# zju3dv/pvnet

Measured on NVIDIA H100. Metric: images/sec (480x640, K=9) backbone+vote, higher is better.
Workload: dtype tf32 (fp32 storage, fp32 accumulate; vote fp32/fp64)

## Files before the change

pvnet_b200/csrc/conv_tc.cu:

```cuda
#include "conv_tc.cuh"
#include "ptx.cuh"

#include <cstdlib>
#include <mutex>
#include <new>

namespace pvnet {

struct ConvGeom {
    int Ho, Wo;
    int tiles_x, tiles_y, total_m_tiles;
    int TH, TW;
    int taps, cin_chunks, cin_pad;
    int Cout, BN;
    int out_cs, out_co;
    int res_cs, res_co;
    int act;
    int round_out;
    signed char tap_map[9];
    short tap_ox[9], tap_oy[9];
    int n_items;
    int stages;
};

struct AMaps {
    CUtensorMap m[4];
};

constexpr int CONV_THREADS = 288;
constexpr int CONV_KC = 32;
constexpr int CONV_A_BYTES = 128 * CONV_KC * 4;

template <int BN, bool MC>
__global__ void __launch_bounds__(CONV_THREADS, 1)
    k_conv_tap(const __grid_constant__ AMaps amaps, const __grid_constant__ CUtensorMap tmB, const __grid_constant__ ConvGeom g,
               const float *__restrict__ bias, const float *__restrict__ res, float *__restrict__ out)
{
    constexpr int B_BYTES = BN * CONV_KC * 4;
    constexpr int STAGE_BYTES = CONV_A_BYTES + B_BYTES;
    const int STAGES = g.stages;
    extern __shared__ uint8_t smem_raw[];
    uint8_t *smem = reinterpret_cast<uint8_t *>((reinterpret_cast<uintptr_t>(smem_raw) + 1023) & ~uintptr_t(1023));
    uint64_t *full = reinterpret_cast<uint64_t *>(smem + (size_t)STAGES * STAGE_BYTES);
    uint64_t *empty = full + STAGES;

    const int warp = threadIdx.x >> 5, lane = threadIdx.x & 31;
    const int tiles_per_img = g.tiles_x * g.tiles_y;
    const int n_tiles_n = g.Cout / BN;
    const int nkb = g.taps * g.cin_chunks;
    const uint32_t crank = MC ? ptx::cluster_ctarank() : 0u;
    const int unit = MC ? (int)blockIdx.x >> 1 : (int)blockIdx.x, nunits = MC ? (int)gridDim.x >> 1 : (int)gridDim.x;
    auto item_tile = [&](int item, int &m_tile, int &n0) {
        const int mi = item / n_tiles_n;
        n0 = (item - mi * n_tiles_n) * BN;
        m_tile = MC ? min(2 * mi + (int)crank, g.total_m_tiles - 1) : mi;
    };

    if (threadIdx.x == 0) {
        for (int s = 0; s < STAGES; ++s) {
            ptx::mbar_init(&full[s], 1);
            ptx::mbar_init(&empty[s], MC ? 16 : 8);
        }
        ptx::fence_barrier_init();
    }
    __syncthreads();
    if (MC) ptx::cluster_sync();

    if (warp == 8) {
        if (lane == 0) {
            int s = 0;
            uint32_t ph = 0;
            for (int item = unit; item < g.n_items; item += nunits) {
                int m_tile, n0;
                item_tile(item, m_tile, n0);
                const int img = m_tile / tiles_per_img;
                const int trem = m_tile - img * tiles_per_img;
                const int tyi = trem / g.tiles_x, txi = trem - tyi * g.tiles_x;
                const int y0 = tyi * g.TH, x0 = txi * g.TW;
                for (int tap = 0; tap < g.taps; ++tap)
                    for (int cc = 0; cc < g.cin_chunks; ++cc) {
                        ptx::mbar_wait(&empty[s], ph ^ 1u);
                        ptx::mbar_arrive_expect_tx(&full[s], (uint32_t)STAGE_BYTES);
                        uint8_t *sa = smem + (size_t)s * STAGE_BYTES;
                        ptx::tma_load_4d(sa, &amaps.m[g.tap_map[tap]], &full[s], cc * CONV_KC, x0 + g.tap_ox[tap],
                                         y0 + g.tap_oy[tap], img);
                        if (MC)
                            ptx::tma_load_2d_mc(sa + CONV_A_BYTES + crank * (B_BYTES / 2), &tmB, &full[s],
                                                tap * g.cin_pad + cc * CONV_KC, n0 + (int)crank * (BN / 2), (uint16_t)0x3);
                        else
                            ptx::tma_load_2d(sa + CONV_A_BYTES, &tmB, &full[s], tap * g.cin_pad + cc * CONV_KC, n0);
                        if (++s == STAGES) {
                            s = 0;
                            ph ^= 1u;
                        }
                    }
            }
        }
    } else {
        const int wg = warp >> 2, wq = warp & 3;
        const int g8 = lane >> 2, t4 = lane & 3;
        const uint32_t smem_u = ptx::smem_u32(smem);
        auto release = [&](int st) {
            ptx::mbar_arrive(&empty[st]);
            if (MC) ptx::mbar_arrive_cluster(&empty[st], crank ^ 1u);
        };
        int s = 0;
        uint32_t ph = 0;
        for (int item = unit; item < g.n_items; item += nunits) {
            float acc[BN / 2];
#pragma unroll
            for (int i = 0; i < BN / 2; ++i) acc[i] = 0.f;
            int prev = -1;
            for (int kb = 0; kb < nkb; ++kb) {
                ptx::mbar_wait(&full[s], ph);
                const uint32_t sa = smem_u + (uint32_t)s * (uint32_t)STAGE_BYTES;
                const uint64_t adesc = ptx::make_kmajor_desc(sa + (uint32_t)(wg * 64 * 128), 128);
                const uint64_t bdesc = ptx::make_kmajor_desc(sa + (uint32_t)CONV_A_BYTES, 128);
                ptx::wgmma_fence();
#pragma unroll
                for (int k = 0; k < CONV_KC / 8; ++k)
                    ptx::Wgmma<BN>::ss(acc, adesc + (uint64_t)(2 * k), bdesc + (uint64_t)(2 * k), (kb | k) != 0 ? 1u : 0u);
                ptx::wgmma_commit();
                ptx::wgmma_wait<1>();
                ptx::fence_regs(acc);
                if (prev >= 0 && lane == 0) release(prev);
                prev = s;
                if (++s == STAGES) {
                    s = 0;
                    ph ^= 1u;
                }
            }
            ptx::wgmma_wait<0>();
            ptx::fence_regs(acc);
            if (lane == 0) release(prev);

            int m_tile, n0;
            item_tile(item, m_tile, n0);
            const int img = m_tile / tiles_per_img;
            const int trem = m_tile - img * tiles_per_img;
            const int tyi = trem / g.tiles_x, txi = trem - tyi * g.tiles_x;
            bool ok[2];
            float *optr[2];
            const float *rptr[2];
#pragma unroll
            for (int h = 0; h < 2; ++h) {
                const int m = wg * 64 + wq * 16 + g8 + 8 * h;
                const int y = tyi * g.TH + m / g.TW, x = txi * g.TW + m % g.TW;
                ok[h] = y < g.Ho && x < g.Wo;
                const size_t pix = ok[h] ? ((size_t)img * g.Ho + y) * g.Wo + x : 0;
                optr[h] = out + pix * g.out_cs + g.out_co + n0;
                rptr[h] = res ? res + pix * g.res_cs + g.res_co + n0 : nullptr;
            }
            constexpr int JC = BN == 256 ? 2 : (BN / 8 < 8 ? BN / 8 : 8);
#pragma unroll
            for (int j0 = 0; j0 < BN / 8; j0 += JC) {
                float2 bv[JC], rv[2][JC];
#pragma unroll
                for (int jj = 0; jj < JC; ++jj)
                    bv[jj] = __ldg(reinterpret_cast<const float2 *>(bias + n0 + 8 * (j0 + jj) + 2 * t4));
                if (res) {
#pragma unroll
                    for (int h = 0; h < 2; ++h)
#pragma unroll
                        for (int jj = 0; jj < JC; ++jj)
                            rv[h][jj] = ok[h] ? __ldg(reinterpret_cast<const float2 *>(rptr[h] + 8 * (j0 + jj) + 2 * t4))
                                              : make_float2(0.f, 0.f);
                }
#pragma unroll
                for (int h = 0; h < 2; ++h) {
                    if (!ok[h]) continue;
#pragma unroll
                    for (int jj = 0; jj < JC; ++jj) {
                        const int j = j0 + jj;
                        float2 v = make_float2(acc[4 * j + 2 * h] + bv[jj].x, acc[4 * j + 2 * h + 1] + bv[jj].y);
                        if (res) {
                            v.x += rv[h][jj].x;
                            v.y += rv[h][jj].y;
                        }
                        v.x = epi_act(v.x, g.act, g.round_out);
                        v.y = epi_act(v.y, g.act, g.round_out);
                        *reinterpret_cast<float2 *>(optr[h] + 8 * j + 2 * t4) = v;
                    }
                }
            }
        }
    }
    if (MC) ptx::cluster_sync();
}

typedef CUresult (*EncodeTiledFn)(CUtensorMap *, CUtensorMapDataType, cuuint32_t, void *, const cuuint64_t *,
                                  const cuuint64_t *, const cuuint32_t *, const cuuint32_t *, CUtensorMapInterleave,
                                  CUtensorMapSwizzle, CUtensorMapL2promotion, CUtensorMapFloatOOBfill);

static EncodeTiledFn encode_fn()
{
    static EncodeTiledFn fn = nullptr;
    static std::once_flag once;
    std::call_once(once, [] {
        void *p = nullptr;
        cudaDriverEntryPointQueryResult q;
        if (cudaGetDriverEntryPoint("cuTensorMapEncodeTiled", &p, cudaEnableDefault, &q) == cudaSuccess &&
            q == cudaDriverEntryPointSuccess)
            fn = reinterpret_cast<EncodeTiledFn>(p);
    });
    return fn;
}

int tma_encode(CUtensorMap *m, const void *base, int rank, const cuuint64_t *dims, const cuuint64_t *strides_bytes,
               const cuuint32_t *box, int swizzle_bytes)
{
    EncodeTiledFn fn = encode_fn();
    if (!fn) {
        set_error("cuTensorMapEncodeTiled entry point unavailable");
        return PVNET_E_CUDA;
    }
    cuuint32_t estr[5] = {1, 1, 1, 1, 1};
    const CUtensorMapSwizzle sw = swizzle_bytes == 128 ? CU_TENSOR_MAP_SWIZZLE_128B
                                  : swizzle_bytes == 64 ? CU_TENSOR_MAP_SWIZZLE_64B
                                                        : CU_TENSOR_MAP_SWIZZLE_32B;
    CUresult r = fn(m, CU_TENSOR_MAP_DATA_TYPE_FLOAT32, (cuuint32_t)rank, const_cast<void *>(base), dims,
                    strides_bytes, box, estr, CU_TENSOR_MAP_INTERLEAVE_NONE, sw, CU_TENSOR_MAP_L2_PROMOTION_L2_128B,
                    CU_TENSOR_MAP_FLOAT_OOB_FILL_NONE);
    if (r == CUDA_ERROR_INVALID_CONTEXT || r == CUDA_ERROR_NOT_INITIALIZED) {
        cudaFree(nullptr);
        r = fn(m, CU_TENSOR_MAP_DATA_TYPE_FLOAT32, (cuuint32_t)rank, const_cast<void *>(base), dims, strides_bytes, box, estr,
               CU_TENSOR_MAP_INTERLEAVE_NONE, sw, CU_TENSOR_MAP_L2_PROMOTION_L2_128B, CU_TENSOR_MAP_FLOAT_OOB_FILL_NONE);
    }
    if (r != CUDA_SUCCESS) {
        set_error("cuTensorMapEncodeTiled failed with CUresult %d (rank %d, dims %llu %llu, box %u %u, swizzle %d)",
                  (int)r, rank, (unsigned long long)dims[0], (unsigned long long)dims[1], box[0], box[1],
                  swizzle_bytes);
        return PVNET_E_CUDA;
    }
    return PVNET_OK;
}

struct ConvPlan {
    AMaps amaps;
    CUtensorMap tmB;
    ConvGeom g;
    dim3 grid;
    size_t smem;
    int mc;
    const float *bias, *res;
    float *out;
};

int g_conv_persist = 1;
int g_conv_mc = 0;

int conv_plan(const ConvDesc &d, ConvPlan *p)
{
    PV_CHECK_ARG(d.in && d.w && d.bias && d.out, "conv: null pointer");
    PV_CHECK_ARG(!d.in2, "conv: a second input source is only supported by the column kernel");
    PV_CHECK_ARG(d.ksize == 1 || d.ksize == 3, "conv: kernel size %d unsupported", d.ksize);
    PV_CHECK_ARG(d.stride == 1 || d.stride == 2, "conv: stride %d unsupported", d.stride);
    PV_CHECK_ARG(d.stride == 1 || (d.dilation == 1 && d.H % 2 == 0 && d.W % 2 == 0),
                 "conv: stride 2 needs dilation 1 and even H,W");
    PV_CHECK_ARG(d.Cout % 32 == 0, "conv: Cout %d must be a multiple of 32", d.Cout);
    PV_CHECK_ARG(d.in_cs % 4 == 0 && d.in_co % 4 == 0 && d.out_cs % 4 == 0 && d.out_co % 4 == 0,
                 "conv: channel strides/offsets must be multiples of 4 floats");
    PV_CHECK_ARG(!d.res || (d.res_cs % 4 == 0 && d.res_co % 4 == 0), "conv: residual stride/offset alignment");
    PV_CHECK_ARG(((uintptr_t)d.in % 16 == 0) && ((uintptr_t)d.w % 16 == 0) && ((uintptr_t)d.out % 16 == 0) &&
                     ((uintptr_t)d.bias % 16 == 0),
                 "conv: pointers must be 16-byte aligned");
    PV_CHECK_ARG(d.Cin % 4 == 0, "conv: Cin %d must be a multiple of 4", d.Cin);
    const int kc = CONV_KC;
    ConvGeom &g = p->g;
    g.Ho = d.H / d.stride;
    g.Wo = d.W / d.stride;
    g.TH = 8;
    g.TW = 16;
    g.tiles_x = (g.Wo + g.TW - 1) / g.TW;
    g.tiles_y = (g.Ho + g.TH - 1) / g.TH;
    g.total_m_tiles = g.tiles_x * g.tiles_y * d.b;
    g.taps = d.ksize * d.ksize;
    g.cin_chunks = (d.Cin + kc - 1) / kc;
    g.cin_pad = g.cin_chunks * kc;
    g.Cout = d.Cout;
    {
        const long long sms = sm_count() > 0 ? sm_count() : 1;
        long long best = -1;
        for (int bn = 256; bn >= 32; bn >>= 1) {
            if (d.Cout % bn) continue;
            const long long items = (long long)g.total_m_tiles * (d.Cout / bn);
            const long long cost = (items + sms - 1) / sms * (CONV_A_BYTES + bn * kc * 4);
            if (best < 0 || cost < best) {
                best = cost;
                g.BN = bn;
            }
        }
    }
    g.out_cs = d.out_cs;
    g.out_co = d.out_co;
    g.res_cs = d.res_cs;
    g.res_co = d.res_co;
    g.act = d.act;
    g.round_out = d.round_out;
    const int pad = d.dilation * (d.ksize - 1) / 2;
    for (int t = 0; t < g.taps; ++t) {
        const int kh = t / d.ksize, kw = t - kh * d.ksize;
        if (d.stride == 1) {
            g.tap_map[t] = 0;
            g.tap_ox[t] = (short)(kw * d.dilation - pad);
            g.tap_oy[t] = (short)(kh * d.dilation - pad);
        } else {
            const int dy = kh - pad, dx = kw - pad;
            const int py = dy & 1, px = dx & 1;
            g.tap_map[t] = (signed char)(py * 2 + px);
            g.tap_oy[t] = (short)((dy - py) / 2);
            g.tap_ox[t] = (short)((dx - px) / 2);
        }
    }
    const int swz = kc * 4;
    const int nplanes = d.stride == 2 ? 4 : 1;
    for (int pl = 0; pl < nplanes; ++pl) {
        const int py = pl >> 1, px = pl & 1;
        const float *base = d.in + d.in_co + ((size_t)py * d.W + px) * d.in_cs;
        cuuint64_t dims[4] = {(cuuint64_t)d.Cin, (cuuint64_t)(d.W / d.stride), (cuuint64_t)(d.H / d.stride),
                              (cuuint64_t)d.b};
        cuuint64_t strides[3] = {(cuuint64_t)d.stride * d.in_cs * 4, (cuuint64_t)d.stride * d.W * d.in_cs * 4,
                                 (cuuint64_t)d.H * d.W * d.in_cs * 4};
        cuuint32_t box[4] = {(cuuint32_t)kc, (cuuint32_t)g.TW, (cuuint32_t)g.TH, 1};
        int rc = tma_encode(&p->amaps.m[pl], base, 4, dims, strides, box, swz);
        if (rc) return rc;
    }
    for (int pl = nplanes; pl < 4; ++pl) p->amaps.m[pl] = p->amaps.m[0];
    {
        cuuint64_t dims[2] = {(cuuint64_t)g.taps * g.cin_pad, (cuuint64_t)d.Cout};
        cuuint64_t strides[1] = {(cuuint64_t)g.taps * g.cin_pad * 4};
        p->mc = g_conv_mc;
        cuuint32_t box[2] = {(cuuint32_t)kc, (cuuint32_t)(p->mc ? g.BN / 2 : g.BN)};
        int rc = tma_encode(&p->tmB, d.w, 2, dims, strides, box, swz);
        if (rc) return rc;
    }
    const size_t stage_b = (size_t)CONV_A_BYTES + (size_t)g.BN * kc * 4;
    int st = (int)((227 * 1024 - 1024 - 256) / stage_b);
    if (st > 8) st = 8;
    g.stages = st;
    p->smem = 1024 + (size_t)st * stage_b + 256;
    const int m_units = p->mc ? (g.total_m_tiles + 1) / 2 : g.total_m_tiles;
    g.n_items = m_units * (d.Cout / g.BN);
    long long units = g_conv_persist ? (long long)sm_count() / (p->mc ? 2 : 1) : (long long)g.n_items;
    if (units > g.n_items) units = g.n_items;
    p->grid = dim3((unsigned)(units * (p->mc ? 2 : 1)));
    p->bias = d.bias;
    p->res = d.res;
    p->out = d.out;
    return PVNET_OK;
}

template <int BN, bool MC>
int conv_launch_t(const ConvPlan &p, cudaStream_t s)
{
    const cudaError_t attr_err = ensure_max_smem((const void *)k_conv_tap<BN, MC>, 227 * 1024);
    PV_CUDA(attr_err);
    cudaLaunchConfig_t cfg = {};
    cfg.gridDim = p.grid;
    cfg.blockDim = dim3(CONV_THREADS);
    cfg.dynamicSmemBytes = p.smem;
    cfg.stream = s;
    cudaLaunchAttribute attr[1];
    attr[0].id = cudaLaunchAttributeClusterDimension;
    attr[0].val.clusterDim.x = MC ? 2 : 1;
    attr[0].val.clusterDim.y = 1;
    attr[0].val.clusterDim.z = 1;
    cfg.attrs = attr;
    cfg.numAttrs = MC ? 1 : 0;
    PV_CUDA(cudaLaunchKernelEx(&cfg, k_conv_tap<BN, MC>, p.amaps, p.tmB, p.g, p.bias, p.res, p.out));
    PV_LAUNCHED("k_conv_tap");
    return PVNET_OK;
}

int conv_launch(const ConvPlan &p, cudaStream_t s)
{
    if (p.mc) {
        if (p.g.BN == 256) return conv_launch_t<256, true>(p, s);
        if (p.g.BN == 128) return conv_launch_t<128, true>(p, s);
        if (p.g.BN == 64) return conv_launch_t<64, true>(p, s);
        return conv_launch_t<32, true>(p, s);
    }
    if (p.g.BN == 256) return conv_launch_t<256, false>(p, s);
    if (p.g.BN == 128) return conv_launch_t<128, false>(p, s);
    if (p.g.BN == 64) return conv_launch_t<64, false>(p, s);
    return conv_launch_t<32, false>(p, s);
}

size_t conv_plan_size() { return sizeof(ConvPlan); }
int conv_plan_at(const ConvDesc &d, void *storage) { return conv_plan(d, new (storage) ConvPlan()); }
int conv_launch_at(const void *storage, cudaStream_t s) { return conv_launch(*static_cast<const ConvPlan *>(storage), s); }

}

extern "C" {

int pvnet_conv_set_multicast(int on)
{
    PV_CHECK_ARG(on == 0 || on == 1, "multicast mode must be 0 or 1");
    pvnet::g_conv_mc = on;
    return PVNET_OK;
}

int pvnet_conv_set_persistent(int on)
{
    pvnet::g_conv_persist = on ? 1 : 0;
    return PVNET_OK;
}

int pvnet_conv2d_nhwc(const float *in, int in_cs, int in_co, int Cin, const float *w_packed, const float *bias,
                      const float *res, int res_cs, int res_co, float *out, int out_cs, int out_co, int Cout, int b,
                      int H, int W, int ksize, int stride, int dilation, int act, int round_out,
                      pvnet_stream_t stream)
{
    pvnet::ConvDesc d{in, in_cs, in_co, Cin, w_packed, bias, res, res_cs, res_co, out, out_cs, out_co, Cout,
                      b, H, W, ksize, stride, dilation, act, round_out};
    const bool col = pvnet::g_conv_mode == 2 || (pvnet::g_conv_mode == 0 && pvnet::conv_col_eligible(d));
    if (col) {
        alignas(64) unsigned char storage[2048];
        static_assert(sizeof(storage) >= 1024, "plan storage");
        if (pvnet::conv_col_plan_size() > sizeof(storage)) {
            pvnet::set_error("column plan larger than its stack storage");
            return PVNET_E_STATE;
        }
        int rc = pvnet::conv_col_plan_at(d, nullptr, storage);
        if (rc) return rc;
        return pvnet::conv_col_launch_at(storage, (cudaStream_t)stream);
    }
    pvnet::ConvPlan plan;
    int rc = pvnet::conv_plan(d, &plan);
    if (rc) return rc;
    return pvnet::conv_launch(plan, (cudaStream_t)stream);
}

}
```

pvnet_b200/csrc/ptx.cuh:

```cuda
#pragma once
#include <cstdint>
#include <cuda.h>
#include <cuda_runtime.h>

namespace ptx {

__device__ __forceinline__ uint32_t smem_u32(const void *p)
{
    return static_cast<uint32_t>(__cvta_generic_to_shared(p));
}

__device__ __forceinline__ bool elect_one()
{
    uint32_t pred = 0;
    asm volatile(
        "{\n\t"
        ".reg .pred P1;\n\t"
        "elect.sync _|P1, 0xffffffff;\n\t"
        "selp.b32 %0, 1, 0, P1;\n\t"
        "}\n"
        : "=r"(pred));
    return pred != 0;
}

__device__ __forceinline__ void mbar_init(uint64_t *bar, uint32_t count)
{
    asm volatile("mbarrier.init.shared::cta.b64 [%0], %1;" ::"r"(smem_u32(bar)), "r"(count));
}
__device__ __forceinline__ void fence_barrier_init()
{
    asm volatile("fence.mbarrier_init.release.cluster;" ::: "memory");
}
__device__ __forceinline__ void fence_proxy_async()
{
    asm volatile("fence.proxy.async.shared::cta;" ::: "memory");
}
__device__ __forceinline__ void mbar_arrive_expect_tx(uint64_t *bar, uint32_t bytes)
{
    asm volatile("mbarrier.arrive.expect_tx.shared::cta.b64 _, [%0], %1;" ::"r"(smem_u32(bar)), "r"(bytes)
                 : "memory");
}
__device__ __forceinline__ void mbar_arrive(uint64_t *bar)
{
    asm volatile("mbarrier.arrive.shared::cta.b64 _, [%0];" ::"r"(smem_u32(bar)) : "memory");
}
__device__ __forceinline__ bool mbar_try_wait(uint64_t *bar, uint32_t parity)
{
    uint32_t ok;
    asm volatile(
        "{\n\t"
        ".reg .pred P1;\n\t"
        "mbarrier.try_wait.parity.shared::cta.b64 P1, [%1], %2;\n\t"
        "selp.b32 %0, 1, 0, P1;\n\t"
        "}\n"
        : "=r"(ok)
        : "r"(smem_u32(bar)), "r"(parity)
        : "memory");
    return ok != 0;
}
__device__ __forceinline__ void mbar_wait(uint64_t *bar, uint32_t parity)
{
    while (!mbar_try_wait(bar, parity)) {
    }
}

__device__ __forceinline__ void prefetch_tensormap(const CUtensorMap *m)
{
    asm volatile("prefetch.tensormap [%0];" ::"l"(reinterpret_cast<uint64_t>(m)) : "memory");
}
__device__ __forceinline__ void tma_load_4d(void *smem_dst, const CUtensorMap *m, uint64_t *bar, int c0, int c1,
                                            int c2, int c3)
{
    asm volatile(
        "cp.async.bulk.tensor.4d.shared::cluster.global.mbarrier::complete_tx::bytes [%0], [%1, {%3, %4, %5, %6}], [%2];"
        ::"r"(smem_u32(smem_dst)), "l"(reinterpret_cast<uint64_t>(m)), "r"(smem_u32(bar)), "r"(c0), "r"(c1), "r"(c2),
        "r"(c3)
        : "memory");
}
__device__ __forceinline__ void tma_load_2d(void *smem_dst, const CUtensorMap *m, uint64_t *bar, int c0, int c1)
{
    asm volatile(
        "cp.async.bulk.tensor.2d.shared::cluster.global.mbarrier::complete_tx::bytes [%0], [%1, {%3, %4}], [%2];"
        ::"r"(smem_u32(smem_dst)), "l"(reinterpret_cast<uint64_t>(m)), "r"(smem_u32(bar)), "r"(c0), "r"(c1)
        : "memory");
}

__device__ __forceinline__ void tma_store_4d(const CUtensorMap *m, const void *smem_src, int c0, int c1, int c2, int c3)
{
    asm volatile("cp.async.bulk.tensor.4d.global.shared::cta.bulk_group [%0, {%2, %3, %4, %5}], [%1];" ::"l"(
                     reinterpret_cast<uint64_t>(m)),
                 "r"(smem_u32(smem_src)), "r"(c0), "r"(c1), "r"(c2), "r"(c3)
                 : "memory");
}
__device__ __forceinline__ void tma_store_commit() { asm volatile("cp.async.bulk.commit_group;" ::: "memory"); }
__device__ __forceinline__ void tma_store_wait_read() { asm volatile("cp.async.bulk.wait_group.read 0;" ::: "memory"); }
__device__ __forceinline__ void tma_store_wait_read1() { asm volatile("cp.async.bulk.wait_group.read 1;" ::: "memory"); }
__device__ __forceinline__ void tma_store_wait_all() { asm volatile("cp.async.bulk.wait_group 0;" ::: "memory"); }
__device__ __forceinline__ void sts128(uint32_t addr, float4 v)
{
    asm volatile("st.shared.v4.f32 [%0], {%1, %2, %3, %4};" ::"r"(addr), "f"(v.x), "f"(v.y), "f"(v.z), "f"(v.w) : "memory");
}
__device__ __forceinline__ float4 lds128(uint32_t addr)
{
    float4 v;
    asm volatile("ld.shared.v4.f32 {%0, %1, %2, %3}, [%4];" : "=f"(v.x), "=f"(v.y), "=f"(v.z), "=f"(v.w) : "r"(addr) : "memory");
    return v;
}
__device__ __forceinline__ void sts64(uint32_t addr, float2 v)
{
    asm volatile("st.shared.v2.f32 [%0], {%1, %2};" ::"r"(addr), "f"(v.x), "f"(v.y) : "memory");
}
__device__ __forceinline__ void sts32(uint32_t addr, float v) { asm volatile("st.shared.f32 [%0], %1;" ::"r"(addr), "f"(v) : "memory"); }
__device__ __forceinline__ float lds32(uint32_t addr)
{
    float v;
    asm volatile("ld.shared.f32 %0, [%1];" : "=f"(v) : "r"(addr) : "memory");
    return v;
}
__device__ __forceinline__ void sts8(uint32_t addr, uint32_t v) { asm volatile("st.shared.u8 [%0], %1;" ::"r"(addr), "r"(v) : "memory"); }
__device__ __forceinline__ uint32_t lds8(uint32_t addr)
{
    uint32_t v;
    asm volatile("ld.shared.u8 %0, [%1];" : "=r"(v) : "r"(addr) : "memory");
    return v;
}
__device__ __forceinline__ void tma_store_4d_u32(const CUtensorMap *m, uint32_t smem_src, int c0, int c1, int c2, int c3)
{
    asm volatile("cp.async.bulk.tensor.4d.global.shared::cta.bulk_group [%0, {%2, %3, %4, %5}], [%1];" ::"l"(
                     reinterpret_cast<uint64_t>(m)),
                 "r"(smem_src), "r"(c0), "r"(c1), "r"(c2), "r"(c3)
                 : "memory");
}
__device__ __forceinline__ void named_bar_sync(int id, int nthreads)
{
    asm volatile("bar.sync %0, %1;" ::"r"(id), "r"(nthreads) : "memory");
}

__device__ __forceinline__ uint32_t cluster_ctarank()
{
    uint32_t r;
    asm volatile("mov.u32 %0, %%cluster_ctarank;" : "=r"(r));
    return r;
}
__device__ __forceinline__ void cluster_sync()
{
    asm volatile("barrier.cluster.arrive.release.aligned;\n\tbarrier.cluster.wait.acquire.aligned;" ::: "memory");
}
__device__ __forceinline__ uint32_t mapa(const void *p, uint32_t rank)
{
    uint32_t r;
    asm volatile("mapa.shared::cluster.u32 %0, %1, %2;" : "=r"(r) : "r"(smem_u32(p)), "r"(rank));
    return r;
}
__device__ __forceinline__ float ld_cluster_f32(uint32_t addr)
{
    float v;
    asm volatile("ld.shared::cluster.f32 %0, [%1];" : "=f"(v) : "r"(addr) : "memory");
    return v;
}
__device__ __forceinline__ unsigned long long ld_cluster_u64(uint32_t addr)
{
    unsigned long long v;
    asm volatile("ld.shared::cluster.u64 %0, [%1];" : "=l"(v) : "r"(addr) : "memory");
    return v;
}
__device__ __forceinline__ void mbar_arrive_cluster(uint64_t *bar, uint32_t rank)
{
    asm volatile(
        "{\n\t.reg .b32 ra;\n\tmapa.shared::cluster.u32 ra, %0, %1;\n\t"
        "mbarrier.arrive.release.cluster.shared::cluster.b64 _, [ra];\n\t}" ::"r"(smem_u32(bar)), "r"(rank)
        : "memory");
}
__device__ __forceinline__ void tma_load_2d_mc(void *smem_dst, const CUtensorMap *m, uint64_t *bar, int c0, int c1,
                                               uint16_t cta_mask)
{
    asm volatile(
        "cp.async.bulk.tensor.2d.shared::cluster.global.mbarrier::complete_tx::bytes.multicast::cluster"
        " [%0], [%1, {%4, %5}], [%2], %3;"
        ::"r"(smem_u32(smem_dst)), "l"(reinterpret_cast<uint64_t>(m)), "r"(smem_u32(bar)), "h"(cta_mask), "r"(c0),
        "r"(c1)
        : "memory");
}

__device__ __forceinline__ void wgmma_fence() { asm volatile("wgmma.fence.sync.aligned;" ::: "memory"); }
__device__ __forceinline__ void wgmma_commit() { asm volatile("wgmma.commit_group.sync.aligned;" ::: "memory"); }
template <int N>
__device__ __forceinline__ void wgmma_wait() { asm volatile("wgmma.wait_group.sync.aligned %0;" ::"n"(N) : "memory"); }
template <int R>
__device__ __forceinline__ void fence_regs(float (&d)[R])
{
#pragma unroll
    for (int i = 0; i < R; ++i) asm volatile("" : "+f"(d[i])::"memory");
}

template <int N>
struct Wgmma;
template <>
struct Wgmma<32> {
    __device__ __forceinline__ static void ss(float (&d)[16], uint64_t adesc, uint64_t bdesc, uint32_t accumulate)
    {
        asm volatile(
            "{\n\t.reg .pred p;\n\tsetp.ne.b32 p, %18, 0;\n\t"
            "wgmma.mma_async.sync.aligned.m64n32k8.f32.tf32.tf32 {%0, %1, %2, %3, %4, %5, %6, %7, %8, %9, %10, %11, %12, %13, %14, %15}, %16, %17, p, 1, 1;\n\t}\n"
            : "+f"(d[0]), "+f"(d[1]), "+f"(d[2]), "+f"(d[3]), "+f"(d[4]), "+f"(d[5]), "+f"(d[6]), "+f"(d[7]), "+f"(d[8]), "+f"(d[9]), "+f"(d[10]), "+f"(d[11]), "+f"(d[12]), "+f"(d[13]), "+f"(d[14]), "+f"(d[15])
            : "l"(adesc), "l"(bdesc), "r"(accumulate));
    }
    __device__ __forceinline__ static void rs(float (&d)[16], const uint32_t (&a)[4], uint64_t bdesc, uint32_t accumulate)
    {
        asm volatile(
            "{\n\t.reg .pred p;\n\tsetp.ne.b32 p, %21, 0;\n\t"
            "wgmma.mma_async.sync.aligned.m64n32k8.f32.tf32.tf32 {%0, %1, %2, %3, %4, %5, %6, %7, %8, %9, %10, %11, %12, %13, %14, %15}, {%16, %17, %18, %19}, %20, p, 1, 1;\n\t}\n"
            : "+f"(d[0]), "+f"(d[1]), "+f"(d[2]), "+f"(d[3]), "+f"(d[4]), "+f"(d[5]), "+f"(d[6]), "+f"(d[7]), "+f"(d[8]), "+f"(d[9]), "+f"(d[10]), "+f"(d[11]), "+f"(d[12]), "+f"(d[13]), "+f"(d[14]), "+f"(d[15])
            : "r"(a[0]), "r"(a[1]), "r"(a[2]), "r"(a[3]), "l"(bdesc), "r"(accumulate));
    }
};

template <>
struct Wgmma<64> {
    __device__ __forceinline__ static void ss(float (&d)[32], uint64_t adesc, uint64_t bdesc, uint32_t accumulate)
    {
        asm volatile(
            "{\n\t.reg .pred p;\n\tsetp.ne.b32 p, %34, 0;\n\t"
            "wgmma.mma_async.sync.aligned.m64n64k8.f32.tf32.tf32 {%0, %1, %2, %3, %4, %5, %6, %7, %8, %9, %10, %11, %12, %13, %14, %15, %16, %17, %18, %19, %20, %21, %22, %23, %24, %25, %26, %27, %28, %29, %30, %31}, %32, %33, p, 1, 1;\n\t}\n"
            : "+f"(d[0]), "+f"(d[1]), "+f"(d[2]), "+f"(d[3]), "+f"(d[4]), "+f"(d[5]), "+f"(d[6]), "+f"(d[7]), "+f"(d[8]), "+f"(d[9]), "+f"(d[10]), "+f"(d[11]), "+f"(d[12]), "+f"(d[13]), "+f"(d[14]), "+f"(d[15]), "+f"(d[16]), "+f"(d[17]), "+f"(d[18]), "+f"(d[19]), "+f"(d[20]), "+f"(d[21]), "+f"(d[22]), "+f"(d[23]), "+f"(d[24]), "+f"(d[25]), "+f"(d[26]), "+f"(d[27]), "+f"(d[28]), "+f"(d[29]), "+f"(d[30]), "+f"(d[31])
            : "l"(adesc), "l"(bdesc), "r"(accumulate));
    }
    __device__ __forceinline__ static void rs(float (&d)[32], const uint32_t (&a)[4], uint64_t bdesc, uint32_t accumulate)
    {
        asm volatile(
            "{\n\t.reg .pred p;\n\tsetp.ne.b32 p, %37, 0;\n\t"
            "wgmma.mma_async.sync.aligned.m64n64k8.f32.tf32.tf32 {%0, %1, %2, %3, %4, %5, %6, %7, %8, %9, %10, %11, %12, %13, %14, %15, %16, %17, %18, %19, %20, %21, %22, %23, %24, %25, %26, %27, %28, %29, %30, %31}, {%32, %33, %34, %35}, %36, p, 1, 1;\n\t}\n"
            : "+f"(d[0]), "+f"(d[1]), "+f"(d[2]), "+f"(d[3]), "+f"(d[4]), "+f"(d[5]), "+f"(d[6]), "+f"(d[7]), "+f"(d[8]), "+f"(d[9]), "+f"(d[10]), "+f"(d[11]), "+f"(d[12]), "+f"(d[13]), "+f"(d[14]), "+f"(d[15]), "+f"(d[16]), "+f"(d[17]), "+f"(d[18]), "+f"(d[19]), "+f"(d[20]), "+f"(d[21]), "+f"(d[22]), "+f"(d[23]), "+f"(d[24]), "+f"(d[25]), "+f"(d[26]), "+f"(d[27]), "+f"(d[28]), "+f"(d[29]), "+f"(d[30]), "+f"(d[31])
            : "r"(a[0]), "r"(a[1]), "r"(a[2]), "r"(a[3]), "l"(bdesc), "r"(accumulate));
    }
};

template <>
struct Wgmma<128> {
    __device__ __forceinline__ static void ss(float (&d)[64], uint64_t adesc, uint64_t bdesc, uint32_t accumulate)
    {
        asm volatile(
            "{\n\t.reg .pred p;\n\tsetp.ne.b32 p, %66, 0;\n\t"
            "wgmma.mma_async.sync.aligned.m64n128k8.f32.tf32.tf32 {%0, %1, %2, %3, %4, %5, %6, %7, %8, %9, %10, %11, %12, %13, %14, %15, %16, %17, %18, %19, %20, %21, %22, %23, %24, %25, %26, %27, %28, %29, %30, %31, %32, %33, %34, %35, %36, %37, %38, %39, %40, %41, %42, %43, %44, %45, %46, %47, %48, %49, %50, %51, %52, %53, %54, %55, %56, %57, %58, %59, %60, %61, %62, %63}, %64, %65, p, 1, 1;\n\t}\n"
            : "+f"(d[0]), "+f"(d[1]), "+f"(d[2]), "+f"(d[3]), "+f"(d[4]), "+f"(d[5]), "+f"(d[6]), "+f"(d[7]), "+f"(d[8]), "+f"(d[9]), "+f"(d[10]), "+f"(d[11]), "+f"(d[12]), "+f"(d[13]), "+f"(d[14]), "+f"(d[15]), "+f"(d[16]), "+f"(d[17]), "+f"(d[18]), "+f"(d[19]), "+f"(d[20]), "+f"(d[21]), "+f"(d[22]), "+f"(d[23]), "+f"(d[24]), "+f"(d[25]), "+f"(d[26]), "+f"(d[27]), "+f"(d[28]), "+f"(d[29]), "+f"(d[30]), "+f"(d[31]), "+f"(d[32]), "+f"(d[33]), "+f"(d[34]), "+f"(d[35]), "+f"(d[36]), "+f"(d[37]), "+f"(d[38]), "+f"(d[39]), "+f"(d[40]), "+f"(d[41]), "+f"(d[42]), "+f"(d[43]), "+f"(d[44]), "+f"(d[45]), "+f"(d[46]), "+f"(d[47]), "+f"(d[48]), "+f"(d[49]), "+f"(d[50]), "+f"(d[51]), "+f"(d[52]), "+f"(d[53]), "+f"(d[54]), "+f"(d[55]), "+f"(d[56]), "+f"(d[57]), "+f"(d[58]), "+f"(d[59]), "+f"(d[60]), "+f"(d[61]), "+f"(d[62]), "+f"(d[63])
            : "l"(adesc), "l"(bdesc), "r"(accumulate));
    }
    __device__ __forceinline__ static void rs(float (&d)[64], const uint32_t (&a)[4], uint64_t bdesc, uint32_t accumulate)
    {
        asm volatile(
            "{\n\t.reg .pred p;\n\tsetp.ne.b32 p, %69, 0;\n\t"
            "wgmma.mma_async.sync.aligned.m64n128k8.f32.tf32.tf32 {%0, %1, %2, %3, %4, %5, %6, %7, %8, %9, %10, %11, %12, %13, %14, %15, %16, %17, %18, %19, %20, %21, %22, %23, %24, %25, %26, %27, %28, %29, %30, %31, %32, %33, %34, %35, %36, %37, %38, %39, %40, %41, %42, %43, %44, %45, %46, %47, %48, %49, %50, %51, %52, %53, %54, %55, %56, %57, %58, %59, %60, %61, %62, %63}, {%64, %65, %66, %67}, %68, p, 1, 1;\n\t}\n"
            : "+f"(d[0]), "+f"(d[1]), "+f"(d[2]), "+f"(d[3]), "+f"(d[4]), "+f"(d[5]), "+f"(d[6]), "+f"(d[7]), "+f"(d[8]), "+f"(d[9]), "+f"(d[10]), "+f"(d[11]), "+f"(d[12]), "+f"(d[13]), "+f"(d[14]), "+f"(d[15]), "+f"(d[16]), "+f"(d[17]), "+f"(d[18]), "+f"(d[19]), "+f"(d[20]), "+f"(d[21]), "+f"(d[22]), "+f"(d[23]), "+f"(d[24]), "+f"(d[25]), "+f"(d[26]), "+f"(d[27]), "+f"(d[28]), "+f"(d[29]), "+f"(d[30]), "+f"(d[31]), "+f"(d[32]), "+f"(d[33]), "+f"(d[34]), "+f"(d[35]), "+f"(d[36]), "+f"(d[37]), "+f"(d[38]), "+f"(d[39]), "+f"(d[40]), "+f"(d[41]), "+f"(d[42]), "+f"(d[43]), "+f"(d[44]), "+f"(d[45]), "+f"(d[46]), "+f"(d[47]), "+f"(d[48]), "+f"(d[49]), "+f"(d[50]), "+f"(d[51]), "+f"(d[52]), "+f"(d[53]), "+f"(d[54]), "+f"(d[55]), "+f"(d[56]), "+f"(d[57]), "+f"(d[58]), "+f"(d[59]), "+f"(d[60]), "+f"(d[61]), "+f"(d[62]), "+f"(d[63])
            : "r"(a[0]), "r"(a[1]), "r"(a[2]), "r"(a[3]), "l"(bdesc), "r"(accumulate));
    }
};

template <>
struct Wgmma<256> {
    __device__ __forceinline__ static void ss(float (&d)[128], uint64_t adesc, uint64_t bdesc, uint32_t accumulate)
    {
        asm volatile(
            "{\n\t.reg .pred p;\n\tsetp.ne.b32 p, %130, 0;\n\t"
            "wgmma.mma_async.sync.aligned.m64n256k8.f32.tf32.tf32 {%0, %1, %2, %3, %4, %5, %6, %7, %8, %9, %10, %11, %12, %13, %14, %15, %16, %17, %18, %19, %20, %21, %22, %23, %24, %25, %26, %27, %28, %29, %30, %31, %32, %33, %34, %35, %36, %37, %38, %39, %40, %41, %42, %43, %44, %45, %46, %47, %48, %49, %50, %51, %52, %53, %54, %55, %56, %57, %58, %59, %60, %61, %62, %63, %64, %65, %66, %67, %68, %69, %70, %71, %72, %73, %74, %75, %76, %77, %78, %79, %80, %81, %82, %83, %84, %85, %86, %87, %88, %89, %90, %91, %92, %93, %94, %95, %96, %97, %98, %99, %100, %101, %102, %103, %104, %105, %106, %107, %108, %109, %110, %111, %112, %113, %114, %115, %116, %117, %118, %119, %120, %121, %122, %123, %124, %125, %126, %127}, %128, %129, p, 1, 1;\n\t}\n"
            : "+f"(d[0]), "+f"(d[1]), "+f"(d[2]), "+f"(d[3]), "+f"(d[4]), "+f"(d[5]), "+f"(d[6]), "+f"(d[7]), "+f"(d[8]), "+f"(d[9]), "+f"(d[10]), "+f"(d[11]), "+f"(d[12]), "+f"(d[13]), "+f"(d[14]), "+f"(d[15]), "+f"(d[16]), "+f"(d[17]), "+f"(d[18]), "+f"(d[19]), "+f"(d[20]), "+f"(d[21]), "+f"(d[22]), "+f"(d[23]), "+f"(d[24]), "+f"(d[25]), "+f"(d[26]), "+f"(d[27]), "+f"(d[28]), "+f"(d[29]), "+f"(d[30]), "+f"(d[31]), "+f"(d[32]), "+f"(d[33]), "+f"(d[34]), "+f"(d[35]), "+f"(d[36]), "+f"(d[37]), "+f"(d[38]), "+f"(d[39]), "+f"(d[40]), "+f"(d[41]), "+f"(d[42]), "+f"(d[43]), "+f"(d[44]), "+f"(d[45]), "+f"(d[46]), "+f"(d[47]), "+f"(d[48]), "+f"(d[49]), "+f"(d[50]), "+f"(d[51]), "+f"(d[52]), "+f"(d[53]), "+f"(d[54]), "+f"(d[55]), "+f"(d[56]), "+f"(d[57]), "+f"(d[58]), "+f"(d[59]), "+f"(d[60]), "+f"(d[61]), "+f"(d[62]), "+f"(d[63]), "+f"(d[64]), "+f"(d[65]), "+f"(d[66]), "+f"(d[67]), "+f"(d[68]), "+f"(d[69]), "+f"(d[70]), "+f"(d[71]), "+f"(d[72]), "+f"(d[73]), "+f"(d[74]), "+f"(d[75]), "+f"(d[76]), "+f"(d[77]), "+f"(d[78]), "+f"(d[79]), "+f"(d[80]), "+f"(d[81]), "+f"(d[82]), "+f"(d[83]), "+f"(d[84]), "+f"(d[85]), "+f"(d[86]), "+f"(d[87]), "+f"(d[88]), "+f"(d[89]), "+f"(d[90]), "+f"(d[91]), "+f"(d[92]), "+f"(d[93]), "+f"(d[94]), "+f"(d[95]), "+f"(d[96]), "+f"(d[97]), "+f"(d[98]), "+f"(d[99]), "+f"(d[100]), "+f"(d[101]), "+f"(d[102]), "+f"(d[103]), "+f"(d[104]), "+f"(d[105]), "+f"(d[106]), "+f"(d[107]), "+f"(d[108]), "+f"(d[109]), "+f"(d[110]), "+f"(d[111]), "+f"(d[112]), "+f"(d[113]), "+f"(d[114]), "+f"(d[115]), "+f"(d[116]), "+f"(d[117]), "+f"(d[118]), "+f"(d[119]), "+f"(d[120]), "+f"(d[121]), "+f"(d[122]), "+f"(d[123]), "+f"(d[124]), "+f"(d[125]), "+f"(d[126]), "+f"(d[127])
            : "l"(adesc), "l"(bdesc), "r"(accumulate));
    }
};

__device__ __forceinline__ float round_tf32(float x)
{
    uint32_t r;
    asm("cvt.rna.tf32.f32 %0, %1;" : "=r"(r) : "f"(x));
    return __uint_as_float(r);
}


__device__ __forceinline__ uint64_t make_kmajor_desc(uint32_t smem_addr, uint32_t swizzle_bytes)
{
    const uint64_t layout = swizzle_bytes == 128 ? 1ull : (swizzle_bytes == 64 ? 2ull : 3ull);
    const uint64_t sbo = (8ull * swizzle_bytes) >> 4;
    return (uint64_t)((smem_addr & 0x3ffff) >> 4) | (1ull << 16) | (sbo << 32) | (layout << 62);
}
__device__ __forceinline__ uint64_t make_kmajor_desc(uint32_t smem_addr, uint32_t swizzle_bytes, uint32_t sbo_bytes)
{
    const uint64_t layout = swizzle_bytes == 128 ? 1ull : (swizzle_bytes == 64 ? 2ull : 3ull);
    return (uint64_t)((smem_addr & 0x3ffff) >> 4) | (1ull << 16) | ((uint64_t)(sbo_bytes >> 4) << 32) | (layout << 62);
}
__device__ __forceinline__ uint32_t swizzle_off(uint32_t off, uint32_t swizzle_bytes)
{
    return off ^ ((off >> 3) & (swizzle_bytes - 16u));
}

}
```

Baseline: 1674.

## Stage conv epilogue through swizzled smem slabs with TMA residual loads and stores

The conv epilogue now writes bias/activation results into double-buffered 32-channel shared-memory slabs and stores them with TMA tensor stores. Previously it used scattered per-thread float2 global stores. Residual inputs are prefetched by the producer warp via TMA into the same slabs, interleaved with its polling of the main pipeline. This should cut uncoalesced global traffic in the epilogue. In exchange it takes shared memory from the mainloop stages, which can reduce pipeline depth, and adds named-barrier syncs per slab plus serialized store waits by thread 0.

```diff
diff --git a/pvnet_b200/csrc/conv_tc.cu b/pvnet_b200/csrc/conv_tc.cu
--- a/pvnet_b200/csrc/conv_tc.cu
+++ b/pvnet_b200/csrc/conv_tc.cu
@@ -30,19 +30,27 @@
 constexpr int CONV_THREADS = 288;
 constexpr int CONV_KC = 32;
 constexpr int CONV_A_BYTES = 128 * CONV_KC * 4;
+constexpr int CONV_SLAB = 32;
+constexpr int CONV_SLAB_BYTES = 128 * CONV_SLAB * 4;
+constexpr int CONV_EPI_BAR = 1;
 
 template <int BN, bool MC>
 __global__ void __launch_bounds__(CONV_THREADS, 1)
-    k_conv_tap(const __grid_constant__ AMaps amaps, const __grid_constant__ CUtensorMap tmB, const __grid_constant__ ConvGeom g,
-               const float *__restrict__ bias, const float *__restrict__ res, float *__restrict__ out)
+    k_conv_tap(const __grid_constant__ AMaps amaps, const __grid_constant__ CUtensorMap tmB,
+               const __grid_constant__ CUtensorMap tmOut, const __grid_constant__ CUtensorMap tmRes,
+               const __grid_constant__ ConvGeom g, const float *__restrict__ bias, const int has_res)
 {
     constexpr int B_BYTES = BN * CONV_KC * 4;
     constexpr int STAGE_BYTES = CONV_A_BYTES + B_BYTES;
+    constexpr int SLABS = BN / CONV_SLAB;
     const int STAGES = g.stages;
     extern __shared__ uint8_t smem_raw[];
     uint8_t *smem = reinterpret_cast<uint8_t *>((reinterpret_cast<uintptr_t>(smem_raw) + 1023) & ~uintptr_t(1023));
-    uint64_t *full = reinterpret_cast<uint64_t *>(smem + (size_t)STAGES * STAGE_BYTES);
+    uint8_t *slab = smem + (size_t)STAGES * STAGE_BYTES;
+    uint64_t *full = reinterpret_cast<uint64_t *>(slab + 2 * CONV_SLAB_BYTES);
     uint64_t *empty = full + STAGES;
+    uint64_t *res_full = empty + STAGES;
+    uint64_t *res_free = res_full + 2;
 
     const int warp = threadIdx.x >> 5, lane = threadIdx.x & 31;
     const int tiles_per_img = g.tiles_x * g.tiles_y;
@@ -61,6 +69,10 @@
             ptx::mbar_init(&full[s], 1);
             ptx::mbar_init(&empty[s], MC ? 16 : 8);
         }
+        for (int i = 0; i < 2; ++i) {
+            ptx::mbar_init(&res_full[i], 1);
+            ptx::mbar_init(&res_free[i], 1);
+        }
         ptx::fence_barrier_init();
     }
     __syncthreads();
@@ -68,6 +80,26 @@
 
     if (warp == 8) {
         if (lane == 0) {
+            int r_item = has_res ? unit : g.n_items, r_slab = 0;
+            uint32_t rq = 0;
+            auto poll_res = [&]() {
+                if (r_item >= g.n_items) return;
+                const uint32_t b = rq & 1u;
+                if (!ptx::mbar_test_wait(&res_free[b], ((rq >> 1) & 1u) ^ 1u)) return;
+                int m_tile, n0;
+                item_tile(r_item, m_tile, n0);
+                const int img = m_tile / tiles_per_img;
+                const int trem = m_tile - img * tiles_per_img;
+                const int tyi = trem / g.tiles_x, txi = trem - tyi * g.tiles_x;
+                ptx::mbar_arrive_expect_tx(&res_full[b], (uint32_t)CONV_SLAB_BYTES);
+                ptx::tma_load_4d(slab + b * CONV_SLAB_BYTES, &tmRes, &res_full[b], n0 + r_slab * CONV_SLAB, txi * g.TW,
+                                 tyi * g.TH, img);
+                ++rq;
+                if (++r_slab == SLABS) {
+                    r_slab = 0;
+                    r_item += nunits;
+                }
+            };
             int s = 0;
             uint32_t ph = 0;
             for (int item = unit; item < g.n_items; item += nunits) {
@@ -79,7 +111,9 @@
                 const int y0 = tyi * g.TH, x0 = txi * g.TW;
                 for (int tap = 0; tap < g.taps; ++tap)
                     for (int cc = 0; cc < g.cin_chunks; ++cc) {
-                        ptx::mbar_wait(&empty[s], ph ^ 1u);
+                        poll_res();
+                        while (!(has_res ? ptx::mbar_test_wait(&empty[s], ph ^ 1u) : ptx::mbar_try_wait(&empty[s], ph ^ 1u)))
+                            poll_res();
                         ptx::mbar_arrive_expect_tx(&full[s], (uint32_t)STAGE_BYTES);
                         uint8_t *sa = smem + (size_t)s * STAGE_BYTES;
                         ptx::tma_load_4d(sa, &amaps.m[g.tap_map[tap]], &full[s], cc * CONV_KC, x0 + g.tap_ox[tap],
@@ -95,6 +129,7 @@
                         }
                     }
             }
+            while (r_item < g.n_items) poll_res();
         }
     } else {
         const int wg = warp >> 2, wq = warp & 3;
@@ -105,7 +140,7 @@
             if (MC) ptx::mbar_arrive_cluster(&empty[st], crank ^ 1u);
         };
         int s = 0;
-        uint32_t ph = 0;
+        uint32_t ph = 0, sq = 0;
         for (int item = unit; item < g.n_items; item += nunits) {
             float acc[BN / 2];
 #pragma unroll
@@ -139,51 +174,51 @@
             const int img = m_tile / tiles_per_img;
             const int trem = m_tile - img * tiles_per_img;
             const int tyi = trem / g.tiles_x, txi = trem - tyi * g.tiles_x;
-            bool ok[2];
-            float *optr[2];
-            const float *rptr[2];
-#pragma unroll
-            for (int h = 0; h < 2; ++h) {
-                const int m = wg * 64 + wq * 16 + g8 + 8 * h;
-                const int y = tyi * g.TH + m / g.TW, x = txi * g.TW + m % g.TW;
-                ok[h] = y < g.Ho && x < g.Wo;
-                const size_t pix = ok[h] ? ((size_t)img * g.Ho + y) * g.Wo + x : 0;
-                optr[h] = out + pix * g.out_cs + g.out_co + n0;
-                rptr[h] = res ? res + pix * g.res_cs + g.res_co + n0 : nullptr;
-            }
-            constexpr int JC = BN == 256 ? 2 : (BN / 8 < 8 ? BN / 8 : 8);
-#pragma unroll
-            for (int j0 = 0; j0 < BN / 8; j0 += JC) {
-                float2 bv[JC], rv[2][JC];
-#pragma unroll
-                for (int jj = 0; jj < JC; ++jj)
-                    bv[jj] = __ldg(reinterpret_cast<const float2 *>(bias + n0 + 8 * (j0 + jj) + 2 * t4));
-                if (res) {
-#pragma unroll
-                    for (int h = 0; h < 2; ++h)
-#pragma unroll
-                        for (int jj = 0; jj < JC; ++jj)
-                            rv[h][jj] = ok[h] ? __ldg(reinterpret_cast<const float2 *>(rptr[h] + 8 * (j0 + jj) + 2 * t4))
-                                              : make_float2(0.f, 0.f);
-                }
-#pragma unroll
-                for (int h = 0; h < 2; ++h) {
-                    if (!ok[h]) continue;
-#pragma unroll
-                    for (int jj = 0; jj < JC; ++jj) {
-                        const int j = j0 + jj;
-                        float2 v = make_float2(acc[4 * j + 2 * h] + bv[jj].x, acc[4 * j + 2 * h + 1] + bv[jj].y);
-                        if (res) {
-                            v.x += rv[h][jj].x;
-                            v.y += rv[h][jj].y;
+            const uint32_t row_off = (uint32_t)((wg * 64 + wq * 16 + g8) * 128 + (t4 & 1) * 8);
+            const uint32_t swz = (uint32_t)(((t4 >> 1) ^ g8) << 4);
+            const uint32_t slab_u = ptx::smem_u32(slab);
+#pragma unroll
+            for (int j = 0; j < SLABS; ++j, ++sq) {
+                const uint32_t b = sq & 1u;
+                const uint32_t base = slab_u + b * (uint32_t)CONV_SLAB_BYTES + row_off;
+                float2 bv[4];
+#pragma unroll
+                for (int jj = 0; jj < 4; ++jj)
+                    bv[jj] = __ldg(reinterpret_cast<const float2 *>(bias + n0 + CONV_SLAB * j + 8 * jj + 2 * t4));
+                if (has_res) ptx::mbar_wait(&res_full[b], (sq >> 1) & 1u);
+                else ptx::named_bar_sync(CONV_EPI_BAR, 256);
+#pragma unroll
+                for (int jj = 0; jj < 4; ++jj)
+#pragma unroll
+                    for (int h = 0; h < 2; ++h) {
+                        const uint32_t addr = base + (uint32_t)(h * 8 * 128) + (swz ^ (uint32_t)(32 * jj));
+                        const int a = 4 * (4 * j + jj) + 2 * h;
+                        float2 v = make_float2(acc[a] + bv[jj].x, acc[a + 1] + bv[jj].y);
+                        if (has_res) {
+                            const float2 r = ptx::lds64(addr);
+                            v.x += r.x;
+                            v.y += r.y;
                         }
                         v.x = epi_act(v.x, g.act, g.round_out);
                         v.y = epi_act(v.y, g.act, g.round_out);
-                        *reinterpret_cast<float2 *>(optr[h] + 8 * j + 2 * t4) = v;
+                        ptx::sts64(addr, v);
+                    }
+                ptx::fence_proxy_async();
+                ptx::named_bar_sync(CONV_EPI_BAR, 256);
+                if (threadIdx.x == 0) {
+                    ptx::tma_store_4d(&tmOut, slab + b * CONV_SLAB_BYTES, n0 + CONV_SLAB * j, txi * g.TW, tyi * g.TH, img);
+                    ptx::tma_store_commit();
+                    if (j == SLABS - 1) ptx::tma_store_wait_read();
+                    else ptx::tma_store_wait_read1();
+                    if (has_res) {
+                        if (j > 0) ptx::mbar_arrive(&res_free[b ^ 1u]);
+                        if (j == SLABS - 1) ptx::mbar_arrive(&res_free[b]);
                     }
                 }
+                __syncwarp();
             }
         }
+        if (threadIdx.x == 0) ptx::tma_store_wait_all();
     }
     if (MC) ptx::cluster_sync();
 }
@@ -238,12 +273,13 @@
 struct ConvPlan {
     AMaps amaps;
     CUtensorMap tmB;
+    CUtensorMap tmOut, tmRes;
     ConvGeom g;
     dim3 grid;
     size_t smem;
     int mc;
-    const float *bias, *res;
-    float *out;
+    const float *bias;
+    int has_res;
 };
 
 int g_conv_persist = 1;
@@ -334,19 +370,34 @@
         int rc = tma_encode(&p->tmB, d.w, 2, dims, strides, box, swz);
         if (rc) return rc;
     }
+    {
+        cuuint64_t dims[4] = {(cuuint64_t)d.Cout, (cuuint64_t)g.Wo, (cuuint64_t)g.Ho, (cuuint64_t)d.b};
+        cuuint32_t box[4] = {(cuuint32_t)CONV_SLAB, (cuuint32_t)g.TW, (cuuint32_t)g.TH, 1};
+        cuuint64_t ostr[3] = {(cuuint64_t)d.out_cs * 4, (cuuint64_t)g.Wo * d.out_cs * 4,
+                              (cuuint64_t)g.Ho * g.Wo * d.out_cs * 4};
+        int rc = tma_encode(&p->tmOut, d.out + d.out_co, 4, dims, ostr, box, CONV_SLAB * 4);
+        if (rc) return rc;
+        p->tmRes = p->tmOut;
+        if (d.res) {
+            PV_CHECK_ARG((uintptr_t)d.res % 16 == 0, "conv: pointers must be 16-byte aligned");
+            cuuint64_t rstr[3] = {(cuuint64_t)d.res_cs * 4, (cuuint64_t)g.Wo * d.res_cs * 4,
+                                  (cuuint64_t)g.Ho * g.Wo * d.res_cs * 4};
+            rc = tma_encode(&p->tmRes, d.res + d.res_co, 4, dims, rstr, box, CONV_SLAB * 4);
+            if (rc) return rc;
+        }
+    }
     const size_t stage_b = (size_t)CONV_A_BYTES + (size_t)g.BN * kc * 4;
-    int st = (int)((227 * 1024 - 1024 - 256) / stage_b);
+    int st = (int)((227 * 1024 - 1024 - 256 - 2 * CONV_SLAB_BYTES) / stage_b);
     if (st > 8) st = 8;
     g.stages = st;
-    p->smem = 1024 + (size_t)st * stage_b + 256;
+    p->smem = 1024 + (size_t)st * stage_b + 2 * CONV_SLAB_BYTES + 256;
     const int m_units = p->mc ? (g.total_m_tiles + 1) / 2 : g.total_m_tiles;
     g.n_items = m_units * (d.Cout / g.BN);
     long long units = g_conv_persist ? (long long)sm_count() / (p->mc ? 2 : 1) : (long long)g.n_items;
     if (units > g.n_items) units = g.n_items;
     p->grid = dim3((unsigned)(units * (p->mc ? 2 : 1)));
     p->bias = d.bias;
-    p->res = d.res;
-    p->out = d.out;
+    p->has_res = d.res != nullptr;
     return PVNET_OK;
 }
 
@@ -367,7 +418,7 @@
     attr[0].val.clusterDim.z = 1;
     cfg.attrs = attr;
     cfg.numAttrs = MC ? 1 : 0;
-    PV_CUDA(cudaLaunchKernelEx(&cfg, k_conv_tap<BN, MC>, p.amaps, p.tmB, p.g, p.bias, p.res, p.out));
+    PV_CUDA(cudaLaunchKernelEx(&cfg, k_conv_tap<BN, MC>, p.amaps, p.tmB, p.tmOut, p.tmRes, p.g, p.bias, p.has_res));
     PV_LAUNCHED("k_conv_tap");
     return PVNET_OK;
 }
diff --git a/pvnet_b200/csrc/ptx.cuh b/pvnet_b200/csrc/ptx.cuh
--- a/pvnet_b200/csrc/ptx.cuh
+++ b/pvnet_b200/csrc/ptx.cuh
@@ -58,6 +58,20 @@
         : "memory");
     return ok != 0;
 }
+__device__ __forceinline__ bool mbar_test_wait(uint64_t *bar, uint32_t parity)
+{
+    uint32_t ok;
+    asm volatile(
+        "{\n\t"
+        ".reg .pred P1;\n\t"
+        "mbarrier.test_wait.parity.shared::cta.b64 P1, [%1], %2;\n\t"
+        "selp.b32 %0, 1, 0, P1;\n\t"
+        "}\n"
+        : "=r"(ok)
+        : "r"(smem_u32(bar)), "r"(parity)
+        : "memory");
+    return ok != 0;
+}
 __device__ __forceinline__ void mbar_wait(uint64_t *bar, uint32_t parity)
 {
     while (!mbar_try_wait(bar, parity)) {
@@ -109,6 +123,12 @@
 __device__ __forceinline__ void sts64(uint32_t addr, float2 v)
 {
     asm volatile("st.shared.v2.f32 [%0], {%1, %2};" ::"r"(addr), "f"(v.x), "f"(v.y) : "memory");
+}
+__device__ __forceinline__ float2 lds64(uint32_t addr)
+{
+    float2 v;
+    asm volatile("ld.shared.v2.f32 {%0, %1}, [%2];" : "=f"(v.x), "=f"(v.y) : "r"(addr) : "memory");
+    return v;
 }
 __device__ __forceinline__ void sts32(uint32_t addr, float v) { asm volatile("st.shared.f32 [%0], %1;" ::"r"(addr), "f"(v) : "memory"); }
 __device__ __forceinline__ float lds32(uint32_t addr)
```

Result: faster. 1733, median of 6 (+3.5%).
